# ucb-bar/Accelerated-TinyMPC

Measured on AMD Instinct MI355X. Metric: MPC solves/sec (batched quadrotor nx=12,nu=4,N=30), higher is better.
Workload: dtype f32; 1 GPU; quadrotor_tracking batched 65536 instances per GPU, cold-start tiny_solve, early_exit (tol 1e-3, max_iter 100); nx=12, nu=4, N=30, instances_per_gpu=65536, instances_total=65536, parallelism=batch-shard x1, world_size_seen=1, backend=none (single process), kernel=tile16<12,4,30,exact>, max_iters=85

## Files before the change

accelerated-tinympc_amd/csrc/admm_tile16.hip:

```cpp
#include "rowlane_math.h"
#include <cstdlib>

namespace tinympc
{

typedef float f32x16 __attribute__((ext_vector_type(16)));
#ifndef TINY_T16_ABLATE
#define TINY_T16_ABLATE 0
#endif
#ifndef TINY_T16_CQ
#define TINY_T16_CQ 1
#endif
#ifndef TINY_T16_BADDR
#define TINY_T16_BADDR 1
#endif
#ifndef TINY_T16_PADTAB
#define TINY_T16_PADTAB 1
#endif
#ifndef TINY_T16_XPOSE
#define TINY_T16_XPOSE 1
#endif
#ifndef TINY_T16_SCHED
#define TINY_T16_SCHED 1
#endif
#ifndef TINY_T16_LINES
#define TINY_T16_LINES 1
#endif
#ifndef TINY_T16_STAMP
#define TINY_T16_STAMP 0
#endif

#if TINY_T16_ABLATE == 1
__device__ __forceinline__ f32x4 t16_fake4(float a, float b, f32x4 c) { c[0] += a; c[1] += b; c[2] += a; c[3] += b; return c; }
#define TINY_MFMA4(a, b, c) t16_fake4((a), (b), (c))
#define TINY_MFMA1(a, b, c) __builtin_amdgcn_mfma_f32_16x16x1f32((a), (b), (c), 0, 0, 0)
#else
#define TINY_MFMA4(a, b, c) __builtin_amdgcn_mfma_f32_16x16x4f32((a), (b), (c), 0, 0, 0)
#define TINY_MFMA1(a, b, c) __builtin_amdgcn_mfma_f32_16x16x1f32((a), (b), (c), 0, 0, 0)
#endif

template <int V>
__device__ __forceinline__ void gather12(float (&t)[12], const f32x16 &p0, const f32x16 &p1, const f32x16 &p2)
{
#pragma unroll
    for (int b = 0; b < 4; b++)
    {
        t[b] = p0[4 * b + V];
        t[4 + b] = p1[4 * b + V];
        t[8 + b] = p2[4 * b + V];
    }
}
template <int V>
__device__ __forceinline__ void gather4(float (&t)[4], const f32x16 &p)
{
#pragma unroll
    for (int b = 0; b < 4; b++) t[b] = p[4 * b + V];
}

typedef float f32x2 __attribute__((ext_vector_type(2)));
template <int B>
__device__ __forceinline__ f32x4 blk(const f32x16 &p) { return __builtin_shufflevector(p, p, 4 * B, 4 * B + 1, 4 * B + 2, 4 * B + 3); }
__device__ __forceinline__ void gather12v(f32x4 (&t)[12], const f32x16 &p0, const f32x16 &p1, const f32x16 &p2)
{
    t[0] = blk<0>(p0); t[1] = blk<1>(p0); t[2] = blk<2>(p0); t[3] = blk<3>(p0);
    t[4] = blk<0>(p1); t[5] = blk<1>(p1); t[6] = blk<2>(p1); t[7] = blk<3>(p1);
    t[8] = blk<0>(p2); t[9] = blk<1>(p2); t[10] = blk<2>(p2); t[11] = blk<3>(p2);
}
__device__ __forceinline__ void gather4v(f32x4 (&t)[4], const f32x16 &p)
{
    t[0] = blk<0>(p); t[1] = blk<1>(p); t[2] = blk<2>(p); t[3] = blk<3>(p);
}
template <int LO, int CNT, int NN>
__device__ __forceinline__ f32x4 tree_sum4(const f32x4 (&t)[NN])
{
    if constexpr (CNT == 1) return t[LO];
    else
    {
        constexpr int H = CNT / 2;
        return tree_sum4<LO, H>(t) + tree_sum4<LO + H, CNT - H>(t);
    }
}
template <int PLO, int PCNT, int L, int NN>
__device__ __forceinline__ f32x4 ptree_sum4(const f32x4 (&t)[NN])
{
    if constexpr (PCNT == 1) return t[4 * PLO + L];
    else
    {
        constexpr int H = PCNT / 2;
        return ptree_sum4<PLO, H, L>(t) + ptree_sum4<PLO + H, PCNT - H, L>(t);
    }
}
template <int PLAN, int NN>
__device__ __forceinline__ f32x4 reduce4(const f32x4 (&t)[NN])
{
    if constexpr (NN == 1) return t[0];
    else if constexpr (PLAN == PLAN_SEQ)
    {
        f32x4 acc = t[0];
#pragma unroll
        for (int k = 1; k < NN; k++) acc = acc + t[k];
        return acc;
    }
    else if constexpr (PLAN == PLAN_TREE) return tree_sum4<0, NN>(t);
    else
    {
        static_assert(NN % 4 == 0, "packed VEC plan: whole packets only");
        constexpr int NPK = NN / 4;
        const f32x4 s0 = ptree_sum4<0, NPK, 0>(t), s1 = ptree_sum4<0, NPK, 1>(t), s2 = ptree_sum4<0, NPK, 2>(t), s3 = ptree_sum4<0, NPK, 3>(t);
        return (s0 + s2) + (s1 + s3);
    }
}

template <bool EXACT>
struct TileMath
{
    static constexpr int NX = 12, NU = 4;
    using PL = RowPlans<NX, NU>;
    float A1[3], A2, A3[3], A45, AP[3];
    f32x16 negz;

    __device__ __forceinline__ void load(const float *mats, int g, int c)
    {
        const float *m = mats + 4 * (c & 3) + (c >> 2);
#pragma unroll
        for (int ch = 0; ch < 3; ch++)
        {
            A1[ch] = m[(4 * ch + g) * 16];
            A3[ch] = m[(NX + NU + 4 * ch + g) * 16];
            AP[ch] = m[(2 * NX + 2 * NU + 1 + 4 * ch + g) * 16];
        }
        A2 = m[(NX + g) * 16];
        A45 = m[(2 * NX + NU + g) * 16];
#pragma unroll
        for (int e = 0; e < 16; e++) negz[e] = -0.f;
    }

    struct InFlight
    {
        f32x16 p0, p1, p2, pk;
        f32x4 acc;
    };

    __device__ __forceinline__ void lqr_issue(const float (&s)[3], InFlight &F) const
    {
        if constexpr (EXACT)
        {
            F.p0 = TINY_MFMA1(A1[0], s[0], negz); F.p1 = TINY_MFMA1(A1[1], s[1], negz); F.p2 = TINY_MFMA1(A1[2], s[2], negz);
        }
        else
        {
            f32x4 acc = {-0.f, -0.f, -0.f, -0.f};
            acc = TINY_MFMA4(A1[0], s[0], acc);
            acc = TINY_MFMA4(A1[1], s[1], acc);
            F.acc = TINY_MFMA4(A1[2], s[2], acc);
        }
    }
    __device__ __forceinline__ void lqr_finish(const InFlight &F, float di, float &un, float (&xn)[3]) const
    {
        if constexpr (EXACT)
        {
            static_assert(PL::FWD_XA == PL::FWD_U, "x rows and the u row of a lane are summed in one order (both SEQ for nx = 12, nu = 4)");
            f32x4 t[12];
            gather12v(t, F.p0, F.p1, F.p2);
            const f32x4 acc = reduce4<PL::FWD_XA>(t);
            un = -acc[3] - di;
            const f32x16 pb = TINY_MFMA1(A2, un, negz);
            f32x4 t2[4];
            gather4v(t2, pb);
            const f32x4 xn4 = acc + reduce4<PL::FWD_XB>(t2);
            xn[0] = xn4[0]; xn[1] = xn4[1]; xn[2] = xn4[2];
        }
        else
        {
            un = F.acc[3] - di;
            const f32x4 acc = TINY_MFMA4(A2, un, F.acc);
            xn[0] = acc[0]; xn[1] = acc[1]; xn[2] = acc[2];
        }
    }
    __device__ __forceinline__ void lqr(const float (&s)[3], float di, float &un, float (&xn)[3]) const
    {
        InFlight F;
        lqr_issue(s, F);
        lqr_finish(F, di, un, xn);
    }

    __device__ __forceinline__ void riccati_issue(const float (&p)[3], const f32x4 &lin, InFlight &F) const
    {
        if constexpr (EXACT)
        {
            F.p0 = TINY_MFMA1(A3[0], p[0], negz); F.p1 = TINY_MFMA1(A3[1], p[1], negz); F.p2 = TINY_MFMA1(A3[2], p[2], negz);
            F.pk = TINY_MFMA1(A45, lin[3], negz);
        }
        else
        {
            f32x4 acc = lin;
            acc = TINY_MFMA4(A3[0], p[0], acc);
            acc = TINY_MFMA4(A3[1], p[1], acc);
            F.acc = TINY_MFMA4(A3[2], p[2], acc);
        }
    }
    __device__ __forceinline__ void riccati_finish(const InFlight &F, const f32x4 &lin, float (&pn)[3], float &dd) const
    {
        if constexpr (EXACT)
        {
            f32x4 t4[12];
            gather12v(t4, F.p0, F.p1, F.p2);
            const f32x4 wv = lin + reduce4<PL::BWD_PA>(t4);
            float t[12];
            gather12<3>(t, F.p0, F.p1, F.p2);
            const float wv3 = lin[3] + reduce<PL::BWD_TMP>(t);
            const f32x16 pq = TINY_MFMA1(A45, wv3, negz);
            f32x4 tk4[4];
            gather4v(tk4, F.pk);
            const f32x4 pn4 = wv - reduce4<PL::BWD_PK>(tk4);
            pn[0] = pn4[0]; pn[1] = pn4[1]; pn[2] = pn4[2];
            float tk[4];
            gather4<3>(tk, pq); dd = reduce<PL::BWD_D>(tk);
        }
        else
        {
            const f32x4 nz = {-0.f, -0.f, -0.f, -0.f};
            const f32x4 dq = TINY_MFMA4(A45, F.acc[3], nz);
            const f32x4 acc = TINY_MFMA4(A45, lin[3], F.acc);
            pn[0] = acc[0]; pn[1] = acc[1]; pn[2] = acc[2];
            dd = dq[3];
        }
    }
    __device__ __forceinline__ void riccati(const float (&p)[3], const f32x4 &lin, float (&pn)[3], float &dd) const
    {
        InFlight F;
        riccati_issue(p, lin, F);
        riccati_finish(F, lin, pn, dd);
    }

    __device__ __forceinline__ void terminal(const float (&xr)[3], float (&pt)[3]) const
    {
        if constexpr (EXACT)
        {
            const f32x16 p0 = TINY_MFMA1(AP[0], xr[0], negz), p1 = TINY_MFMA1(AP[1], xr[1], negz), p2 = TINY_MFMA1(AP[2], xr[2], negz);
            float t[12];
            gather12<0>(t, p0, p1, p2); pt[0] = -reduce<PL::TERM>(t);
            gather12<1>(t, p0, p1, p2); pt[1] = -reduce<PL::TERM>(t);
            gather12<2>(t, p0, p1, p2); pt[2] = -reduce<PL::TERM>(t);
        }
        else
        {
            f32x4 acc = {-0.f, -0.f, -0.f, -0.f};
            acc = TINY_MFMA4(AP[0], xr[0], acc);
            acc = TINY_MFMA4(AP[1], xr[1], acc);
            acc = TINY_MFMA4(AP[2], xr[2], acc);
            pt[0] = -acc[0]; pt[1] = -acc[1]; pt[2] = -acc[2];
        }
    }
};

__device__ __forceinline__ float tile_inst_max(float v)
{
    v = fmaxf(v, __shfl_xor(v, 16));
    v = fmaxf(v, __shfl_xor(v, 32));
    return v;
}

__device__ __forceinline__ void acc_put(float &dst, float val) { asm volatile("v_accvgpr_write_b32 %0, %1" : "+a"(dst) : "v"(val)); }
__device__ __forceinline__ float acc_get(const float &src)
{
    float r;
    asm volatile("v_accvgpr_read_b32 %0, %1" : "=v"(r) : "a"(src));
    return r;
}
__device__ __forceinline__ void acc_init(float &dst, float val) { asm volatile("v_accvgpr_write_b32 %0, %1" : "=a"(dst) : "v"(val)); }

typedef __attribute__((address_space(3))) float4 lds_float4;
__device__ __forceinline__ void masked_forward_update(unsigned long long m, float (&a)[4], const f32x4 &tp, float (&bo)[4], const f32x4 &old,
                                                      unsigned sn_addr, const f32x4 &t)
{
    unsigned long long sx;
    asm volatile("s_and_saveexec_b64 %[sx], %[m]\n\t"
                 "v_sub_f32 %[a0], %[p0], %[t0]\n\tv_sub_f32 %[a1], %[p1], %[t1]\n\tv_sub_f32 %[a2], %[p2], %[t2]\n\tv_sub_f32 %[a3], %[p3], %[t3]\n\t"
                 "v_accvgpr_write_b32 %[b0], %[o0]\n\tv_accvgpr_write_b32 %[b1], %[o1]\n\tv_accvgpr_write_b32 %[b2], %[o2]\n\tv_accvgpr_write_b32 %[b3], %[o3]\n\t"
                 "ds_write_b128 %[ad], %[tv]\n\t"
                 "s_mov_b64 exec, %[sx]"
                 : [sx] "=&s"(sx), [a0] "+v"(a[0]), [a1] "+v"(a[1]), [a2] "+v"(a[2]), [a3] "+v"(a[3]), [b0] "+a"(bo[0]), [b1] "+a"(bo[1]),
                   [b2] "+a"(bo[2]), [b3] "+a"(bo[3])
                 : [m] "s"(m), [p0] "v"(tp[0]), [p1] "v"(tp[1]), [p2] "v"(tp[2]), [p3] "v"(tp[3]), [t0] "v"(t[0]), [t1] "v"(t[1]), [t2] "v"(t[2]),
                   [t3] "v"(t[3]), [o0] "v"(old[0]), [o1] "v"(old[1]), [o2] "v"(old[2]), [o3] "v"(old[3]), [ad] "v"(sn_addr), [tv] "v"(t)
                 : "memory", "scc");
}
__device__ __forceinline__ void masked_backward_update(unsigned long long m, float (&pl)[3], float &dr, const float (&pn)[3], float dd)
{
    unsigned long long sx;
    asm volatile("s_and_saveexec_b64 %[sx], %[m]\n\t"
                 "v_accvgpr_write_b32 %[p0], %[n0]\n\tv_accvgpr_write_b32 %[p1], %[n1]\n\tv_accvgpr_write_b32 %[p2], %[n2]\n\tv_mov_b32 %[d], %[dd]\n\t"
                 "s_mov_b64 exec, %[sx]"
                 : [sx] "=&s"(sx), [p0] "+a"(pl[0]), [p1] "+a"(pl[1]), [p2] "+a"(pl[2]), [d] "+v"(dr)
                 : [m] "s"(m), [n0] "v"(pn[0]), [n1] "v"(pn[1]), [n2] "v"(pn[2]), [dd] "v"(dd)
                 : "scc");
}

__device__ __forceinline__ void masked_restore_slack(unsigned long long m, const float (&bo)[4], unsigned sn_addr)
{
    const f32x4 tv = {acc_get(bo[0]), acc_get(bo[1]), acc_get(bo[2]), acc_get(bo[3])};
    unsigned long long sx;
    asm volatile("s_and_saveexec_b64 %[sx], %[m]\n\t"
                 "ds_write_b128 %[ad], %[tv]\n\t"
                 "s_mov_b64 exec, %[sx]"
                 : [sx] "=&s"(sx)
                 : [m] "s"(m), [ad] "v"(sn_addr), [tv] "v"(tv)
                 : "memory", "scc");
}

template <bool EXACT>
__device__ __forceinline__ f32x4 lin_cost4(const f32x4 &cq, const f32x4 &rho4, const f32x4 &t1)
{
    if constexpr (EXACT) return cq - rho4 * t1;
    else return __builtin_elementwise_fma(-rho4, t1, cq);
}

__device__ __forceinline__ f32x4 t16_transpose4(const f32x4 &r)
{
    typedef unsigned u32x2 __attribute__((ext_vector_type(2)));
    const u32x2 a = __builtin_amdgcn_permlane32_swap(__float_as_uint(r[0]), __float_as_uint(r[2]), false, false);
    const u32x2 b = __builtin_amdgcn_permlane32_swap(__float_as_uint(r[1]), __float_as_uint(r[3]), false, false);
    const u32x2 lo = __builtin_amdgcn_permlane16_swap(a[0], b[0], false, false);
    const u32x2 hi = __builtin_amdgcn_permlane16_swap(a[1], b[1], false, false);
    return f32x4{__uint_as_float(lo[0]), __uint_as_float(lo[1]), __uint_as_float(hi[0]), __uint_as_float(hi[1])};
}

constexpr int TILE16_WAVES = 4;
constexpr int TILE16_MAX_TABLE_ROWS = 512;

__device__ __forceinline__ void t16_pair_lines(const f32x4 &e, const f32x4 &o, f32x4 &lo8, f32x4 &hi8)
{
#pragma unroll
    for (int k = 0; k < 4; k++)
    {
        lo8[k] = __int_as_float(__builtin_amdgcn_update_dpp(__float_as_int(e[k]), __float_as_int(o[k]), 0x128, 0xf, 0xc, false));
        hi8[k] = __int_as_float(__builtin_amdgcn_update_dpp(__float_as_int(o[k]), __float_as_int(e[k]), 0x128, 0xf, 0x3, false));
    }
}

#if TINY_T16_STAMP && !defined(TINY_T16_PI_UNIT)
constexpr int T16_STAMP_TILES = 32;
__device__ unsigned long long *t16_stamp_buf;
__device__ int t16_stamp_slots;
__device__ __forceinline__ void t16_stamp(int wslot, int k, int field, unsigned long long v)
{
    unsigned long long *const buf = t16_stamp_buf;
    if (buf && wslot < t16_stamp_slots && k < T16_STAMP_TILES && (threadIdx.x & 63) == 0) buf[((size_t)wslot * T16_STAMP_TILES + k) * 4 + field] = v;
}
#define T16_STAMP(k, field, v) t16_stamp((int)blockIdx.x * TILE16_WAVES + (int)(threadIdx.x >> 6), (k), (field), (v))
#else
#define T16_STAMP(k, field, v) ((void)0)
#endif

__device__ __forceinline__ void t16_dma_row(unsigned on, const float *sbase, unsigned voff, unsigned lds_dst, float after)
{
    asm volatile("s_cmp_eq_u32 %0, 0\n\ts_cbranch_scc1 1f\n\ts_mov_b32 m0, %3\n\ts_nop 0\n\tglobal_load_lds_dwordx4 %1, %2\n1:"
                 : : "s"(on), "v"(voff), "s"(sbase), "s"(lds_dst), "v"(after) : "memory", "scc");
}
__device__ __forceinline__ void t16_dma_row2(unsigned on, const float *sbase, unsigned voff, unsigned lds_dst, float after0, float after1)
{
    asm volatile("s_cmp_eq_u32 %0, 0\n\ts_cbranch_scc1 1f\n\ts_mov_b32 m0, %3\n\ts_nop 0\n\tglobal_load_lds_dwordx4 %1, %2\n\t"
                 "s_add_u32 m0, m0, 0x3f0\n\ts_nop 0\n\tglobal_load_lds_dwordx4 %1, %2 offset:16\n1:"
                 : : "s"(on), "v"(voff), "s"(sbase), "s"(lds_dst), "v"(after0), "v"(after1) : "memory", "scc");
}
__device__ __forceinline__ void t16_dma_img2(unsigned on, const float *sbase, unsigned voff, unsigned lds_dst, float after0, float after1)
{
    asm volatile("s_cmp_eq_u32 %0, 0\n\ts_cbranch_scc1 1f\n\ts_mov_b32 m0, %3\n\ts_nop 0\n\tglobal_load_lds_dwordx4 %1, %2\n\t"
                 "global_load_lds_dwordx4 %1, %2 offset:1024\n1:"
                 : : "s"(on), "v"(voff), "s"(sbase), "s"(lds_dst), "v"(after0), "v"(after1) : "memory", "scc");
}
__device__ __forceinline__ void t16_wait_vm(int k)
{
    if (k == 0) asm volatile("s_waitcnt vmcnt(0)" ::: "memory");
    else if (k == 1) asm volatile("s_waitcnt vmcnt(1)" ::: "memory");
    else if (k == 2) asm volatile("s_waitcnt vmcnt(2)" ::: "memory");
    else if (k == 3) asm volatile("s_waitcnt vmcnt(3)" ::: "memory");
    else if (k == 4) asm volatile("s_waitcnt vmcnt(4)" ::: "memory");
    else if (k == 5) asm volatile("s_waitcnt vmcnt(5)" ::: "memory");
    else if (k == 6) asm volatile("s_waitcnt vmcnt(6)" ::: "memory");
    else if (k == 7) asm volatile("s_waitcnt vmcnt(7)" ::: "memory");
    else asm volatile("s_waitcnt vmcnt(8)" ::: "memory");
}
constexpr int t16_ring_b(bool XR) { return XR ? 3 : 4; }
constexpr int t16_ring_x(bool BR) { return BR ? 4 : 6; }
constexpr int T16_RING_B = 2048, T16_RING_X = 1024;

template <int N, bool EXACT, bool COLD, bool MPC = false, bool BR = false, bool XR = false>
__global__ __launch_bounds__(WAVE * TILE16_WAVES, 1) void admm_tile16_kernel(const RowParams P)
{
    static_assert(!(MPC && (BR || XR)), "the closed loop on chip is instantiated for batch-shared bounds and a shared / windowed reference");
    constexpr int NX = 12, NU = 4;
    const int lane = threadIdx.x & 63, wv = threadIdx.x >> 6, g = lane >> 4, c = lane & 15;
    const int ntiles = (P.batch + 15) >> 4;
    const float rho = P.rho;
    const f32x4 rho4 = {rho, rho, rho, rho};

    extern __shared__ __attribute__((aligned(16))) float4 lds4_base[];
    float4 *const lds4 = lds4_base;
    float4 *const sn0 = lds4 + wv * (N * WAVE) + lane;
    constexpr int DB = t16_ring_b(XR), DX = t16_ring_x(BR);
    const unsigned ringsB = (P.pi_flags & 1u) ? DB : 2, ringsX = (P.pi_flags & 2u) ? DX : 1;
    const unsigned bnd_f4 = BR ? TILE16_WAVES * ringsB * (T16_RING_B / 16) : 2 * N * 4;
    float4 *const blo = lds4 + TILE16_WAVES * N * WAVE, *const bhi = blo + N * 4, *const tab0 = blo + bnd_f4;
    float4 *const tab = tab0;
    const int tab_rows = P.xref_mode == 1 ? P.table_rows : N;
    const float *tab_src = P.xref_mode == 1 ? P.xref_table : P.xref;
    unsigned dmaB = 0, dmaX = 0;
    if constexpr (BR)
    {
        const unsigned ring = (unsigned)(size_t)(lds_float4 *)blo + wv * (ringsB * T16_RING_B);
        dmaB = __builtin_amdgcn_readfirstlane(ring);
    }
    else
    {
        for (int e = threadIdx.x; e < N * 16; e += WAVE * TILE16_WAVES)
        {
            const float2 lh = reinterpret_cast<const float2 *>(P.bounds)[e];
            const int i = e >> 4, r = e & 15;
            reinterpret_cast<float *>(&blo[i * 4 + (r & 3)])[r >> 2] = lh.x;
            reinterpret_cast<float *>(&bhi[i * 4 + (r & 3)])[r >> 2] = lh.y;
        }
    }
    if constexpr (XR)
    {
        const unsigned ring = (unsigned)(size_t)(lds_float4 *)tab0 + wv * (ringsX * T16_RING_X);
        dmaX = __builtin_amdgcn_readfirstlane(ring);
    }
    else
    {
        for (int e = threadIdx.x; e < (tab_rows + N - 1) * 16; e += WAVE * TILE16_WAVES)
        {
            const int er = (e >> 4) < tab_rows ? (e >> 4) : tab_rows - 1;
            float val = tab_src[er * 16 + (e & 15)];
            if (TINY_T16_CQ) val = -(val * ((e & 15) < NX ? P.mats[(2 * NX + 2 * NU) * 16 + (e & 15)] : 1.f));
            reinterpret_cast<float *>(&tab[(e >> 4) * 4 + (e & 3)])[(e & 15) >> 2] = val;
        }
    }
    if constexpr (!BR || !XR) __syncthreads();

    TileMath<EXACT> M;
    M.load(P.mats, g, c);
    f32x4 qv;
#pragma unroll
    for (int v = 0; v < 3; v++) qv[v] = P.mats[(2 * NX + 2 * NU) * 16 + 4 * v + g];
    qv[3] = 1.f;
    constexpr bool CQ = TINY_T16_CQ && !XR;
    auto cost_of = [&](const f32x4 &xr) { return CQ ? xr : -(xr * qv); };

    constexpr bool DQ = COLD && !MPC;
    int qinc = 1;
    if constexpr (DQ)
    {
        const unsigned tail_stride = (P.pi_flags >> 8) & 0xffu;
        if (tail_stride && (((unsigned)blockIdx.x * TILE16_WAVES + (unsigned)wv) % tail_stride) == 0u) qinc = 0x10000;
        qinc = __builtin_amdgcn_readfirstlane(qinc);
    }
#if TINY_T16_STAMP
    int stamp_k = 0;
#else
    constexpr int stamp_k = 0;
#endif
    for (;;)
    {
    int slot = 0;
    if (lane == 0) slot = atomicAdd(P.n_unsolved + 1, qinc);
    slot = __builtin_amdgcn_readfirstlane(slot);
    T16_STAMP(stamp_k, 0, __builtin_amdgcn_s_memrealtime());
    T16_STAMP(stamp_k, 3, ~0ull);
    if (DQ && ntiles <= 32768)
    {
        const int qh = slot & 0xffff, qt = (int)((unsigned)slot >> 16);
        if (qh + qt >= ntiles) break;
        slot = qinc == 1 ? qh : ntiles - 1 - qt;
    }
    else if (slot >= ntiles) break;
    int ozt;
    asm volatile("s_mov_b32 %0, 0" : "=s"(ozt));
    float4 *const sn = sn0 + ozt;
    float4 *const lds4 = lds4_base + ozt;
    int tile = slot;
    if (P.order) tile = P.order[slot];
    const bool tile_ok = tile >= 0 && tile < ntiles;
    T16_STAMP(stamp_k, 3, (unsigned long long)(unsigned)tile);
    constexpr bool GM = COLD && !MPC && !BR && !XR;
    int inst = tile * 16 + c;
    if constexpr (GM)
        if (P.inst_map) inst = P.inst_map[(tile_ok ? tile : 0) * 16 + c];
    auto in_batch = [&](int i) { return GM ? (unsigned)i < (unsigned)P.batch : i < P.batch; };
    const bool valid = tile_ok && in_batch(inst);
    const int inst_a = valid ? inst : P.batch - 1;

    float a[N][4];
    float dr[N], bo[N][4], pl[N][3];
    auto dual4 = [&](int i) { return f32x4{a[i][0], a[i][1], a[i][2], a[i][3]}; };
    const int ebase = (inst_a * N) * 16 + g;
    int wstart = 0;
    if (P.xref_mode == 1) wstart = P.xref_start[inst_a];
    const bool zdual = COLD || (P.duals_zero != 0);

    if constexpr (COLD)
    {
        const float4 z4 = make_float4(0.f, 0.f, 0.f, 0.f);
#pragma unroll
        for (int i = 0; i < N; i++)
        {
            a[i][0] = a[i][1] = a[i][2] = a[i][3] = 0.f;
#pragma unroll
            for (int v = 0; v < 4; v++) acc_init(bo[i][v], 0.f);
            sn[i * WAVE] = z4;
            acc_init(pl[i][0], 0.f); acc_init(pl[i][1], 0.f); acc_init(pl[i][2], 0.f);
            dr[i] = 0.f;
        }
    }
    else
    {
#pragma unroll
        for (int i = 0; i < N; i++)
        {
            float vzl[4], pdv[4];
#pragma unroll
            for (int v = 0; v < 4; v++)
            {
                const int o = ebase + i * 16 + 4 * v;
                vzl[v] = P.vz[o]; pdv[v] = P.pd[o];
                const float gyv = P.gy[o];
                a[i][v] = zdual ? 0.f : gyv;
                acc_init(bo[i][v], vzl[v]);
            }
            sn[i * WAVE] = make_float4(vzl[0], vzl[1], vzl[2], vzl[3]);
            acc_init(pl[i][0], pdv[0]); acc_init(pl[i][1], pdv[1]); acc_init(pl[i][2], pdv[2]);
            dr[i] = pdv[3];
        }
    }
    float x0[3];
#pragma unroll
    for (int v = 0; v < 3; v++) x0[v] = P.xu[ebase + 4 * v];

    const unsigned onB = BR ? (P.pi_flags & 1u) : 0u, onX = XR ? (P.pi_flags & 2u) : 0u;
    struct PiAddr { unsigned rdB, rdX, voffB, voffX; };
    auto pi_addr = [&](unsigned lane16) {
        const unsigned c16 = lane16 & 0xf0u, gg = lane16 >> 8, cc = c16 >> 4;
        const int ins = tile * 16 + (int)cc;
        const unsigned ia = (unsigned)((tile_ok && ins < P.batch) ? ins : P.batch - 1);
        PiAddr A;
        A.rdB = dmaB + 1024u * (gg >> 1) + c16 + 8u * (gg & 1u);
        A.rdX = dmaX + c16 + 4u * gg;
        A.voffB = ia * P.bounds_inst_stride * 8u + 32u * gg;
        A.voffX = ia * P.xref_inst_stride * 4u + 16u * gg;
        return A;
    };
    const float *const xsrc = P.xref;
    auto load_xref = [&](const float4 *tb, int ws, int i, int gsel = -1) {
        if constexpr (XR)
        {
            unsigned ll = lane;
            asm volatile("" : "+v"(ll));
            const unsigned cc = ll & 15u, gg = ll >> 4;
            if (onX)
            {
                const float *rp = xsrc + ((size_t)((tile_ok ? tile : 0) * N + i) * 64 + cc) * 4 + gg;
                return f32x4{rp[0], rp[64], rp[128], 0.f};
            }
            const int ins = tile * 16 + (int)cc;
            const float *rp = xsrc + (size_t)((tile_ok && ins < P.batch) ? ins : P.batch - 1) * P.xref_inst_stride + i * 16 + gg;
            return f32x4{rp[0], rp[4], rp[8], 0.f};
        }
        else
        {
        int row;
        if constexpr (TINY_T16_PADTAB && !(EXACT && COLD && !MPC && !BR && !XR)) row = (ws < tab_rows - 1 ? ws : tab_rows - 1) + i;
        else { row = ws + i; row = row < tab_rows ? row : tab_rows - 1; }
        const float4 t4 = tb[row * 4 + (gsel >= 0 ? gsel : g)];
        return f32x4{t4.x, t4.y, t4.z, t4.w};
        }
    };
    PiAddr A0 = {0u, 0u, 0u, 0u};
    if constexpr (BR || XR)
    {
        A0 = pi_addr(16u * lane);
        if constexpr (BR) { t16_dma_row2(onB ^ 1u, P.bounds, A0.voffB, dmaB, 0.f, 0.f); t16_dma_row2(onB ^ 1u, P.bounds, A0.voffB + (N - 1) * 128u, dmaB + T16_RING_B, 0.f, 0.f); }
        if constexpr (XR) t16_dma_row((onX >> 1) ^ 1u, xsrc, A0.voffX, dmaX, 0.f);
        asm volatile("s_waitcnt vmcnt(0)" ::: "memory");
    }
    auto load_xref_raw = [&](const float4 *tb, int ws, int i) {
        if constexpr (CQ)
        {
            int row = ws + i;
            row = row < tab_rows ? row : tab_rows - 1;
            const float *rp = tab_src + row * 16 + g;
            return f32x4{rp[0], rp[4], rp[8], 0.f};
        }
        else return load_xref(tb, ws, i);
    };
    float pterm[3];
    {
        const f32x4 xrN4 = load_xref_raw(tab, wstart, N - 1);
        const float xrN[3] = {xrN4[0], xrN4[1], xrN4[2]};
        M.terminal(xrN, pterm);
    }

    int st = TINY_STATUS_UNSOLVED_, itn = 1;
    float r_ps = 0.f, r_pi = 0.f, r_ds = 0.f, r_di = 0.f;
    if (valid && !COLD)
    {
        r_ps = P.res[4 * inst + 0]; r_pi = P.res[4 * inst + 1];
        r_ds = P.res[4 * inst + 2]; r_di = P.res[4 * inst + 3];
    }
    float pN[3] = {0.f, 0.f, 0.f};

    auto backward_sweep = [&](unsigned long long amask, const float4 *snI, const float4 *tabI, int wsI) {
        float p[3] = {pN[0], pN[1], pN[2]};
        auto load_lin = [&](int i, float4 &sl, f32x4 &xr) {
            sl = snI[i * WAVE];
            xr = load_xref(tabI, wsI, i);
        };
        auto make_lin = [&](int i, const float4 &sl, const f32x4 &xr) {
            const f32x4 sni = {sl.x, sl.y, sl.z, sl.w};
            return lin_cost4<EXACT>(cost_of(xr), rho4, sni - dual4(i));
        };
        float4 sl0; f32x4 xr0;
        load_lin(N - 2, sl0, xr0);
        f32x4 lin = make_lin(N - 2, sl0, xr0);
#pragma unroll
        for (int i = N - 2; i >= 0; i--)
        {
            float4 sl_n = make_float4(0.f, 0.f, 0.f, 0.f); f32x4 xr_n = {0.f, 0.f, 0.f, 0.f};
            if (EXACT && i > 0) load_lin(i - 1, sl_n, xr_n);
            typename TileMath<EXACT>::InFlight F;
            M.riccati_issue(p, lin, F);
            if (!EXACT && i > 0) load_lin(i - 1, sl_n, xr_n);
#if TINY_T16_SCHED
            if constexpr (EXACT) __builtin_amdgcn_sched_barrier(0);
#endif
            f32x4 lin_n = lin;
            if (i > 0) lin_n = make_lin(i - 1, sl_n, xr_n);
#if TINY_T16_SCHED
            if constexpr (EXACT) __builtin_amdgcn_sched_barrier(0);
#endif
            float pn[3], dd;
            M.riccati_finish(F, lin, pn, dd);
            masked_backward_update(amask, pl[i], dr[i], pn, dd);
            p[0] = pn[0]; p[1] = pn[1]; p[2] = pn[2];
            lin = lin_n;
        }
    };

    for (int ms = 0;; ++ms)
    {
    if (MPC && ms > 0) { st = TINY_STATUS_UNSOLVED_; itn = 1; }
    bool active = valid && (P.max_iter > 0);
    for (int it = 0; it < P.max_iter; ++it)
    {
        if (!__any(active)) break;
        int oz;
        asm volatile("s_mov_b32 %0, 0" : "=s"(oz));
        float4 *const snI = sn + oz;
        const float4 *bloI = blo + oz, *bhiI = bhi + oz;
        const float4 *const tabI = tab + oz;
        const int wsI = wstart + oz;
        const unsigned long long amask = __ballot(active);
        const unsigned sn_addr = (unsigned)(size_t)(lds_float4 *)snI;
        const unsigned gI = (sn_addr - (unsigned)__builtin_amdgcn_readfirstlane(sn_addr)) >> 8;
        const float4 *const bloG = bloI + gI, *const bhiG = bhiI + gI;
        const float *const bsrcI = P.bounds + oz, *const xsrcI = xsrc + oz;
        unsigned rdBI = 0, rdXI = 0;
        if constexpr (BR || XR)
        {
            const PiAddr AI = pi_addr(sn_addr - __builtin_amdgcn_readfirstlane(sn_addr));
            rdBI = COLD ? AI.rdB : A0.rdB + oz; rdXI = COLD ? AI.rdX : A0.rdX + oz;
        }
        const unsigned sB1 = onB ? T16_RING_B : 0u, sX1 = onX ? T16_RING_X : 0u;
        const unsigned sBlast = onB ? ((N - 1) % DB) * T16_RING_B : T16_RING_B;
        const unsigned lane16I = sn_addr - __builtin_amdgcn_readfirstlane(sn_addr);
        const unsigned timg = (unsigned)(tile_ok ? tile : 0) * (unsigned)N;
        unsigned xw = 0, bw = 0;
        if constexpr (XR) xw = timg * 1024u + (COLD ? lane16I : 16u * lane);
        if constexpr (BR) bw = timg * 2048u + (COLD ? lane16I : 16u * lane);
        auto dma_x = [&](int i, float after) { t16_dma_row(onX, xsrcI, xw + (unsigned)i * 1024u, dmaX + (i % DX) * T16_RING_X, after); };
        auto dma_b = [&](int i, float after0, float after1) { t16_dma_img2(onB, bsrcI, bw + (unsigned)i * 2048u, dmaB + (i % DB) * T16_RING_B, after0, after1); };
        typedef __attribute__((address_space(3))) const f32x2 lds_cfloat2;
        typedef __attribute__((address_space(3))) const float lds_cfloat;
        auto ring_bounds = [&](int i, float4 &lo, float4 &hi) {
            lds_cfloat2 *rp = reinterpret_cast<lds_cfloat2 *>(rdBI + (i == N - 1 ? sBlast : (i % DB) * sB1));
            const f32x2 b0 = rp[0], b1 = rp[32], b2 = rp[64], b3 = rp[96];
            lo = make_float4(b0.x, b1.x, b2.x, b3.x); hi = make_float4(b0.y, b1.y, b2.y, b3.y);
        };
        auto ring_xref = [&](int i) {
            lds_cfloat *rp = reinterpret_cast<lds_cfloat *>(rdXI + (i % DX) * sX1);
            return f32x4{rp[0], rp[64], rp[128], 0.f};
        };
        if constexpr (XR)
        {
#pragma unroll
            for (int k = 0; k < DX; k++) dma_x(N - 2 - k, 0.f);
        }
        if constexpr (BR)
        {
#pragma unroll
            for (int k = 0; k < DB - 1; k++) dma_b(k, 0.f, 0.f);
        }
        float s[3] = {x0[0], x0[1], x0[2]};
        float pri_x = 0.f, dua_x = 0.f, pri_u = 0.f, dua_u = 0.f;
        auto elementwise = [&](int i, const f32x4 &sv, const float4 &lo, const float4 &hi, const float4 &ol) {
            const f32x4 old = {ol.x, ol.y, ol.z, ol.w};
            const f32x4 tp = sv + dual4(i);
            f32x4 t;
            t[0] = __builtin_amdgcn_fmed3f(tp[0], lo.x, hi.x);
            t[1] = __builtin_amdgcn_fmed3f(tp[1], lo.y, hi.y);
            t[2] = __builtin_amdgcn_fmed3f(tp[2], lo.z, hi.z);
            t[3] = __builtin_amdgcn_fmed3f(tp[3], lo.w, hi.w);
            const f32x4 dp = sv - t, dd_ = old - t;
            pri_x = fmaxf(fmaxf(fmaxf(pri_x, fabsf(dp[0])), fabsf(dp[1])), fabsf(dp[2]));
            dua_x = fmaxf(fmaxf(fmaxf(dua_x, fabsf(dd_[0])), fabsf(dd_[1])), fabsf(dd_[2]));
            pri_u = fmaxf(pri_u, fabsf(dp[3]));
            dua_u = fmaxf(dua_u, fabsf(dd_[3]));
            if (i == N - 1)
            {
                const f32x4 an = tp - t;
#pragma unroll
                for (int v = 0; v < 3; v++)
                {
                    const float pn_ = lin_cost<EXACT>(pterm[v], rho, t[v] - an[v]);
                    pN[v] = active ? pn_ : pN[v];
                }
            }
            masked_forward_update(amask, a[i], tp, bo[i], old, sn_addr + i * (WAVE * 16), t);
        };
        f32x4 sv_p = {0.f, 0.f, 0.f, 0.f};
        float4 lo_p = make_float4(0.f, 0.f, 0.f, 0.f), hi_p = lo_p, ol_p = lo_p;
#pragma unroll
        for (int i = 0; i < N; i++)
        {
            float4 lo, hi;
            if constexpr (BR)
            {
                if (i + DB - 1 < N) dma_b(i + DB - 1, lo_p.x, hi_p.w);
                t16_wait_vm(2 * ((N - 1 - i) < (DB - 1) ? (N - 1 - i) : (DB - 1)));
                ring_bounds(i, lo, hi);
            }
            else if constexpr (TINY_T16_BADDR && (COLD || !XR)) { lo = bloG[i * 4]; hi = bhiG[i * 4]; }
            else { lo = bloI[i * 4 + g]; hi = bhiI[i * 4 + g]; }
            const float4 ol = snI[i * WAVE];
            typename TileMath<EXACT>::InFlight F;
            if (i < N - 1) M.lqr_issue(s, F);
#if TINY_T16_SCHED
            if constexpr (EXACT) __builtin_amdgcn_sched_barrier(0);
#endif
            if (i > 0) elementwise(i - 1, sv_p, lo_p, hi_p, ol_p);
            float un = 0.f, xn[3] = {0.f, 0.f, 0.f};
            if (i < N - 1) M.lqr_finish(F, dr[i], un, xn);
            sv_p = f32x4{s[0], s[1], s[2], un};
            lo_p = lo; hi_p = hi; ol_p = ol;
            s[0] = xn[0]; s[1] = xn[1]; s[2] = xn[2];
        }
        elementwise(N - 1, sv_p, lo_p, hi_p, ol_p);
        pri_x = tile_inst_max(pri_x); dua_x = tile_inst_max(dua_x);
        pri_u = tile_inst_max(pri_u); dua_u = tile_inst_max(dua_u);
        bool conv = false;
        if (active)
        {
            itn = it + 1;
            if ((it + 1) % P.check_termination == 0)
            {
                r_ps = pri_x; r_ds = dua_x * rho; r_pi = pri_u; r_di = dua_u * rho;
                conv = (r_ps < P.abs_pri_tol) && (r_pi < P.abs_pri_tol) && (r_ds < P.abs_dua_tol) && (r_di < P.abs_dua_tol);
            }
            if (conv) st = TINY_STATUS_SOLVED_;
        }
        active = active && !conv;
        if (!__any(active)) break;
        if (it == P.max_iter - 1) break;
        {
            float p[3] = {pN[0], pN[1], pN[2]};
            const unsigned long long amask = __ballot(active);
            auto load_lin = [&](int i, float4 &sl, f32x4 &xr) {
                sl = snI[i * WAVE];
                if constexpr (XR) xr = ring_xref(i);
                else xr = load_xref(tabI, wsI, i, TINY_T16_BADDR ? (int)gI : -1);
            };
            auto make_lin = [&](int i, const float4 &sl, const f32x4 &xr) {
                const f32x4 sni = {sl.x, sl.y, sl.z, sl.w};
                return lin_cost4<EXACT>(cost_of(xr), rho4, sni - dual4(i));
            };
            float4 sl0; f32x4 xr0;
            if constexpr (XR) t16_wait_vm(0);
            load_lin(N - 2, sl0, xr0);
            f32x4 lin = make_lin(N - 2, sl0, xr0);
#pragma unroll
            for (int i = N - 2; i >= 0; i--)
            {
                float4 sl_n = make_float4(0.f, 0.f, 0.f, 0.f); f32x4 xr_n = {0.f, 0.f, 0.f, 0.f};
                if constexpr (XR)
                {
                    if (i >= DX) dma_x(i - DX, lin[0]);
                    if (i > 0)
                    {
                        const int hi_j = (i - 2) < (N - 2 - DX) ? (i - 2) : (N - 2 - DX), lo_j = (i - DX) > 0 ? (i - DX) : 0;
                        t16_wait_vm(hi_j >= lo_j ? hi_j - lo_j + 1 : 0);
                    }
                }
                if (EXACT && i > 0) load_lin(i - 1, sl_n, xr_n);
                typename TileMath<EXACT>::InFlight F;
                M.riccati_issue(p, lin, F);
                if (!EXACT && i > 0) load_lin(i - 1, sl_n, xr_n);
#if TINY_T16_SCHED
                if constexpr (EXACT) __builtin_amdgcn_sched_barrier(0);
#endif
                f32x4 lin_n = lin;
                if (i > 0) lin_n = make_lin(i - 1, sl_n, xr_n);
#if TINY_T16_SCHED
                if constexpr (EXACT) __builtin_amdgcn_sched_barrier(0);
#endif
                float pn[3], dd;
                M.riccati_finish(F, lin, pn, dd);
                masked_backward_update(amask, pl[i], dr[i], pn, dd);
                p[0] = pn[0]; p[1] = pn[1]; p[2] = pn[2];
                lin = lin_n;
            }
        }
    }
    if (!MPC || ms + 1 >= P.mpc_steps) break;
    if constexpr (MPC)
    {
        int oz;
        asm volatile("s_mov_b32 %0, 0" : "=s"(oz));
        float4 *const snA = sn + oz;
        const unsigned sn_addr = (unsigned)(size_t)(lds_float4 *)snA;
        const bool solved = st == TINY_STATUS_SOLVED_;
        float un, xn_[3];
        M.lqr(x0, dr[0], un, xn_);
        if (P.u0_traj && valid) P.u0_traj[((long long)ms * P.batch + inst) * NU + g] = un;
        {
            const f32x16 p0 = TINY_MFMA1(M.A1[0], x0[0], M.negz), p1 = TINY_MFMA1(M.A1[1], x0[1], M.negz), p2 = TINY_MFMA1(M.A1[2], x0[2], M.negz);
            const f32x16 pb = TINY_MFMA1(M.A2, un, M.negz);
            f32x4 t[12], t2[4];
            gather12v(t, p0, p1, p2);
            gather4v(t2, pb);
            f32x4 z = {0.f, 0.f, 0.f, 0.f};
            asm volatile("" : "+v"(z));
            f32x4 acc = z + t[0];
#pragma unroll
            for (int k = 1; k < 12; k++) acc = acc + t[k];
            const f32x4 x1 = acc + reduce4<PLAN_SEQ>(t2);
            x0[0] = x1[0]; x0[1] = x1[1]; x0[2] = x1[2];
        }
        const unsigned long long umask = __ballot(valid && !solved);
        if (umask != 0ull) backward_sweep(umask, snA, tab + oz, wstart + oz);
        const unsigned long long smask = __ballot(valid && solved);
#pragma unroll
        for (int i = 0; i < N; i++) masked_restore_slack(smask, bo[i], sn_addr + i * (WAVE * 16));
        if (P.xref_mode == 1)
        {
            wstart += P.window_advance;
            const f32x4 xrN4 = load_xref_raw(tab + oz, wstart, N - 1);
            const float xrN[3] = {xrN4[0], xrN4[1], xrN4[2]};
            M.terminal(xrN, pterm);
        }
#pragma unroll
        for (int i = 0; i < N; i++) a[i][0] = a[i][1] = a[i][2] = a[i][3] = 0.f;
    }
    }
    T16_STAMP(stamp_k, 1, __builtin_amdgcn_s_memrealtime());

    auto inst_of = [&](int col) {
        if constexpr (GM)
        {
            int tl = tile_ok ? tile : 0;
            asm volatile("" : "+s"(tl));
            if (P.inst_map) return P.inst_map[tl * 16 + col];
            return tl * 16 + col;
        }
        else return tile * 16 + col;
    };
    int inst_e = inst, ebase_e = ebase;
    bool valid_e = valid;
    if constexpr (GM)
    {
        unsigned ll = lane;
        asm volatile("" : "+v"(ll));
        inst_e = inst_of((int)(ll & 15u));
        valid_e = tile_ok && in_batch(inst_e);
        ebase_e = ((valid_e ? inst_e : P.batch - 1) * N) * 16 + (int)(ll >> 4);
    }

    if (P.max_iter <= 0)
    {
        if (valid_e && g == 0)
        {
            P.status[inst_e] = TINY_STATUS_UNSOLVED_;
            P.iter[inst_e] = 1;
            atomicAdd(P.n_unsolved, 1);
        }
        T16_STAMP(stamp_k, 2, __builtin_amdgcn_s_memrealtime());
#if TINY_T16_STAMP
        ++stamp_k;
#endif
        continue;
    }

    {
        const bool solved = st == TINY_STATUS_SOLVED_;
        const int c2 = lane >> 2, q2 = lane & 3;
        const int inst2 = inst_of(c2);
        const bool valid2 = tile_ok && in_batch(inst2);
        const int obase2 = ((valid2 ? inst2 : 0) * N) * 16 + 4 * q2;
        typedef float float_ma __attribute__((may_alias));
        typedef f32x4 f32x4_ma __attribute__((may_alias));
        float_ma *const stage_w = reinterpret_cast<float_ma *>(lds4 + wv * (N * WAVE));
        const int rd_off = (c2 * 4 + q2);
        const int obase4 = ebase_e + 3 * g;
        constexpr bool XPOSE = TINY_T16_XPOSE && !(EXACT && !COLD && !MPC);
        auto put = [&](float *dst, int i, const f32x4 &val) {
            if constexpr (XPOSE)
            {
                const f32x4 o = t16_transpose4(val);
                if (valid_e) *reinterpret_cast<f32x4 *>(dst + obase4 + i * 16) = o;
                return;
            }
            float_ma *slot = stage_w + i * (WAVE * 4);
            reinterpret_cast<f32x4_ma *>(slot)[lane] = val;
            asm volatile("" ::: "memory");
            f32x4 o;
            o[0] = slot[rd_off]; o[1] = slot[rd_off + 64]; o[2] = slot[rd_off + 128]; o[3] = slot[rd_off + 192];
            asm volatile("" ::: "memory");
            if (valid2) *reinterpret_cast<f32x4 *>(dst + obase2 + i * 16) = o;
        };
        float s[3] = {x0[0], x0[1], x0[2]};
        if constexpr (XPOSE && TINY_T16_LINES && COLD && !MPC && !BR && !XR)
        {
            auto slack_of = [&](int i) { return reinterpret_cast<const f32x4_ma *>(stage_w + i * (WAVE * 4))[lane]; };
            auto lin_of = [&](int i, const f32x4 &sni) {
                const f32x4 xr = load_xref(tab, wstart, i);
                f32x4 lin = lin_cost4<EXACT>(cost_of(xr), rho4, sni - dual4(i));
                if (i == N - 1) lin[3] = 0.f;
                return lin;
            };
            auto pd_of = [&](int i) { return i == N - 1 ? f32x4{pN[0], pN[1], pN[2], 0.f} : f32x4{acc_get(pl[i][0]), acc_get(pl[i][1]), acc_get(pl[i][2]), dr[i]}; };
            auto vz_of = [&](int i, const f32x4 &sni) {
                f32x4 vzv;
    #pragma unroll
                for (int v = 0; v < 4; v++)
                {
                    const float bov = acc_get(bo[i][v]);
                    vzv[v] = solved ? bov : sni[v];
                }
                return vzv;
            };
            const int instL = inst_of(c & 7), instH = inst_of((c & 7) + 8);
            const bool validL = tile_ok && in_batch(instL), validH = tile_ok && in_batch(instH);
            const int obaseL = (validL ? instL : 0) * (N * 16) + ((c >> 3) << 4) + 4 * g;
            const int offH = ((validH ? instH : 0) - (validL ? instL : 0)) * (N * 16);
            auto put2 = [&](float *dst, int i, const f32x4 &ve, const f32x4 &vo) {
                f32x4 lo8, hi8;
                t16_pair_lines(t16_transpose4(ve), t16_transpose4(vo), lo8, hi8);
                if (validL) *reinterpret_cast<f32x4 *>(dst + obaseL + i * 16) = lo8;
                if (validH) *reinterpret_cast<f32x4 *>(dst + obaseL + offH + i * 16) = hi8;
            };
#pragma unroll
            for (int i = 0; i + 1 < N; i += 2)
            {
                const f32x4 sne = slack_of(i), sno = slack_of(i + 1);
                put2(P.gy, i, dual4(i), dual4(i + 1));
                put2(P.vzn, i, sne, sno);
                put2(P.vz, i, vz_of(i, sne), vz_of(i + 1, sno));
                put2(P.pd, i, pd_of(i), pd_of(i + 1));
                put2(P.qr, i, lin_of(i, sne), lin_of(i + 1, sno));
                float ue = 0.f, xe[3];
                M.lqr(s, dr[i], ue, xe);
                const f32x4 sve = {s[0], s[1], s[2], ue};
                float uo = 0.f, xo[3] = {0.f, 0.f, 0.f};
                if (i + 1 < N - 1) M.lqr(xe, dr[i + 1], uo, xo);
                put2(P.xu, i, sve, f32x4{xe[0], xe[1], xe[2], uo});
                s[0] = xo[0]; s[1] = xo[1]; s[2] = xo[2];
            }
            if constexpr (N % 2 == 1)
            {
                const f32x4 sni = slack_of(N - 1);
                put(P.xu, N - 1, f32x4{s[0], s[1], s[2], 0.f});
                put(P.qr, N - 1, lin_of(N - 1, sni));
                put(P.pd, N - 1, pd_of(N - 1));
                put(P.vz, N - 1, vz_of(N - 1, sni));
                put(P.vzn, N - 1, sni);
                put(P.gy, N - 1, dual4(N - 1));
            }
        }
        else
        {
#pragma unroll
        for (int i = 0; i < N; i++)
        {
            float un = 0.f, xn[3] = {0.f, 0.f, 0.f};
            if (i < N - 1) M.lqr(s, dr[i], un, xn);
            const f32x4 sv = {s[0], s[1], s[2], un};
            const f32x4 sni = reinterpret_cast<const f32x4_ma *>(stage_w + i * (WAVE * 4))[lane];
            const f32x4 xr = load_xref(tab, wstart, i);
            f32x4 lin = lin_cost4<EXACT>(cost_of(xr), rho4, sni - dual4(i));
            if (i == N - 1) lin[3] = 0.f;
            f32x4 pdv = {acc_get(pl[i][0]), acc_get(pl[i][1]), acc_get(pl[i][2]), dr[i]};
            if (i == N - 1) pdv = f32x4{pN[0], pN[1], pN[2], 0.f};
            f32x4 vzv;
#pragma unroll
            for (int v = 0; v < 4; v++)
            {
                const float bov = acc_get(bo[i][v]);
                vzv[v] = solved ? bov : sni[v];
            }
            put(P.xu, i, sv);
            put(P.qr, i, lin);
            put(P.pd, i, pdv);
            put(P.vz, i, vzv);
            put(P.vzn, i, sni);
            put(P.gy, i, dual4(i));
            if constexpr (!XPOSE) reinterpret_cast<f32x4_ma *>(stage_w + i * (WAVE * 4))[lane] = sni;
            s[0] = xn[0]; s[1] = xn[1]; s[2] = xn[2];
        }
        }
        const unsigned long long umask = __ballot(valid_e && !solved);
        if (umask != 0ull)
        {
            const bool unsolved2 = valid2 && ((umask >> c2) & 1ull);
            float p[3] = {pN[0], pN[1], pN[2]};
#pragma unroll
            for (int i = N - 2; i >= 0; i--)
            {
                const f32x4 sni = reinterpret_cast<const f32x4_ma *>(stage_w + i * (WAVE * 4))[lane];
                const f32x4 xr = load_xref(tab, wstart, i);
                const f32x4 lin = lin_cost4<EXACT>(cost_of(xr), rho4, sni - dual4(i));
                float pn[3], dd;
                M.riccati(p, lin, pn, dd);
                if constexpr (XPOSE)
                {
                    const f32x4 o = t16_transpose4(f32x4{pn[0], pn[1], pn[2], dd});
                    if (valid_e && !solved) *reinterpret_cast<f32x4 *>(P.pd + obase4 + i * 16) = o;
                }
                else
                {
                float_ma *slot = stage_w + i * (WAVE * 4);
                reinterpret_cast<f32x4_ma *>(slot)[lane] = f32x4{pn[0], pn[1], pn[2], dd};
                asm volatile("" ::: "memory");
                f32x4 o;
                o[0] = slot[rd_off]; o[1] = slot[rd_off + 64]; o[2] = slot[rd_off + 128]; o[3] = slot[rd_off + 192];
                asm volatile("" ::: "memory");
                if (unsolved2) *reinterpret_cast<f32x4 *>(P.pd + obase2 + i * 16) = o;
                }
                p[0] = pn[0]; p[1] = pn[1]; p[2] = pn[2];
            }
        }
        if (valid_e && g == 0)
        {
            P.res[4 * inst_e + 0] = r_ps; P.res[4 * inst_e + 1] = r_pi;
            P.res[4 * inst_e + 2] = r_ds; P.res[4 * inst_e + 3] = r_di;
            P.status[inst_e] = st;
            P.iter[inst_e] = itn;
            if (!solved) atomicAdd(P.n_unsolved, 1);
        }
        if (MPC && valid)
        {
#pragma unroll
            for (int v = 0; v < 3; v++) P.x0buf[inst * NX + 4 * v + g] = x0[v];
            if (g == 0 && P.xref_mode == 1) P.xref_start[inst] = wstart;
        }
    }
    T16_STAMP(stamp_k, 2, __builtin_amdgcn_s_memrealtime());
#if TINY_T16_STAMP
    ++stamp_k;
#endif
    }
}

#ifdef TINY_T16_ONLY30
#define TINY_FOR_EACH_TILE16(X) X(30)
#else
#define TINY_FOR_EACH_TILE16(X) X(30) X(25) X(20) X(10)
#endif

static inline unsigned t16_tail_stride(const RowParams &P, int ntiles, int nblocks, int asked, bool grouped)
{
    static const int env = [] { const char *e = getenv("TINYMPC_T16_TAIL"); return e ? atoi(e) : -1; }();
    const int forced = asked >= 0 ? asked : env;
    if (ntiles > 32768) return 0u;
    if (forced >= 0) return (P.cold_start && P.mpc_steps <= 1) ? (unsigned)(forced > 255 ? 255 : forced) : 0u;
    if (!P.order || P.mpc_steps > 1 || !P.cold_start) return 0u;
    const int slots = nblocks * TILE16_WAVES;
    if (ntiles < 3 * slots) return 0u;
    if (grouped) return ntiles < 8 * slots ? 12u : 8u;
    return (ntiles >= 4 * slots && ntiles < 8 * slots) ? 4u : 8u;
}

#ifdef TINY_T16_PI_UNIT
size_t tile16_pi_lds_bytes(int N, bool bounds_ring, bool xref_ring, unsigned pi_flags, int table_rows)
{
    const size_t bnd = bounds_ring ? (size_t)TILE16_WAVES * ((pi_flags & 1u) ? t16_ring_b(xref_ring) : 2) * T16_RING_B : (size_t)2 * N * 4 * sizeof(float4);
    const size_t ref = xref_ring ? (size_t)TILE16_WAVES * ((pi_flags & 2u) ? t16_ring_x(bounds_ring) : 1) * T16_RING_X : (size_t)(table_rows + N - 1) * 4 * sizeof(float4);
    return (size_t)TILE16_WAVES * N * WAVE * sizeof(float4) + bnd + ref;
}

hipError_t launch_admm_tile16_pi(int N, bool exact, bool bounds_ring, bool xref_ring, const RowParams &P, hipStream_t stream, int n_cu, int tail)
{
    const int ntiles = (P.batch + 15) / 16;
    if (n_cu <= 0) n_cu = 256;
    const int want = (ntiles + TILE16_WAVES - 1) / TILE16_WAVES, nblocks = want < n_cu ? want : n_cu;
    if (P.mpc_steps > 1 || (!bounds_ring && !xref_ring)) return hipErrorInvalidValue;
    if (P.xref_mode == 1 && P.table_rows < 1) return hipErrorInvalidValue;
    if (!bounds_ring && P.bounds_inst_stride != 0) return hipErrorInvalidValue;
    if (!xref_ring && P.xref_mode != 1 && P.xref_inst_stride != 0) return hipErrorInvalidValue;
    if (xref_ring && P.xref_mode == 1) return hipErrorInvalidValue;
    const size_t lds = tile16_pi_lds_bytes(N, bounds_ring, xref_ring, P.pi_flags, P.xref_mode == 1 ? P.table_rows : N);
    if (lds > 160 * 1024) return hipErrorInvalidValue;
    RowParams Q = P;
    Q.inst_map = nullptr;
    Q.pi_flags = (Q.pi_flags & 0xffu) | (t16_tail_stride(P, ntiles, nblocks, tail, false) << 8);
#define TINY_TILE16_PI_LAUNCH3(NN, EX, BRR, XRR)                                                                           \
    {                                                                                                                      \
        auto kern = P.cold_start ? admm_tile16_kernel<NN, EX, true, false, BRR, XRR> : admm_tile16_kernel<NN, EX, false, false, BRR, XRR>; \
        hipError_t e = hipFuncSetAttribute((const void *)kern, hipFuncAttributeMaxDynamicSharedMemorySize, (int)lds);      \
        if (e != hipSuccess) return e;                                                                                     \
        hipLaunchKernelGGL(kern, dim3(nblocks), dim3(WAVE * TILE16_WAVES), lds, stream, Q);                                \
        return hipGetLastError();                                                                                          \
    }
#define TINY_TILE16_PI_LAUNCH(NN, EX)                                             \
    {                                                                             \
// ... 97 lines not shown
```

Before: 48.00 million solves/s.

## Hoist exec masking to whole forward/backward sweeps in cold exact path

For the exact cold-start non-MPC kernel, the active-lane exec mask is now narrowed once around the whole forward and backward sweeps instead of being saved and restored inside every per-step masked update. The per-step updates become plain asm without exec toggling, and the last add of d_i is fused into the backward-update asm. Explicit s_waitcnt plus sched barriers are inserted ahead of LDS consumers, and the reference-table row clamp is changed for this path. The intent is to remove scalar exec save/restore overhead from the hot loop. The risk is that compiler-generated code inside the narrowed region also runs only on active lanes, and the hand-placed waits may over-serialise.

```diff
diff --git a/accelerated-tinympc_amd/csrc/admm_tile16.hip b/accelerated-tinympc_amd/csrc/admm_tile16.hip
--- a/accelerated-tinympc_amd/csrc/admm_tile16.hip
+++ b/accelerated-tinympc_amd/csrc/admm_tile16.hip
@@ -16,6 +16,12 @@
 #endif
 #ifndef TINY_T16_PADTAB
 #define TINY_T16_PADTAB 1
+#endif
+#ifndef TINY_T16_HEADPAD
+#define TINY_T16_HEADPAD 1
+#endif
+#ifndef TINY_T16_HEADWAIT
+#define TINY_T16_HEADWAIT 1
 #endif
 #ifndef TINY_T16_XPOSE
 #define TINY_T16_XPOSE 1
@@ -199,7 +205,8 @@
             F.acc = TINY_MFMA4(A3[2], p[2], acc);
         }
     }
-    __device__ __forceinline__ void riccati_finish(const InFlight &F, const f32x4 &lin, float (&pn)[3], float &dd) const
+    template <bool SPLIT = false>
+    __device__ __forceinline__ void riccati_finish(const InFlight &F, const f32x4 &lin, float (&pn)[3], float &dd, float *ddb = nullptr) const
     {
         if constexpr (EXACT)
         {
@@ -215,7 +222,13 @@
             const f32x4 pn4 = wv - reduce4<PL::BWD_PK>(tk4);
             pn[0] = pn4[0]; pn[1] = pn4[1]; pn[2] = pn4[2];
             float tk[4];
-            gather4<3>(tk, pq); dd = reduce<PL::BWD_D>(tk);
+            gather4<3>(tk, pq);
+            if constexpr (SPLIT)
+            {
+                static_assert(!SPLIT || PL::BWD_D == PLAN_SEQ, "d_i is summed sequentially: ((t0 + t1) + t2) + t3");
+                dd = (tk[0] + tk[1]) + tk[2]; *ddb = tk[3];
+            }
+            else dd = reduce<PL::BWD_D>(tk);
         }
         else
         {
@@ -297,6 +310,36 @@
                  : "scc");
 }
 
+#pragma clang diagnostic push
+#pragma clang diagnostic ignored "-Winline-asm"
+__device__ __forceinline__ unsigned long long exec_narrow(unsigned long long m)
+{
+    unsigned long long sx;
+    asm volatile("s_and_saveexec_b64 %0, %1" : "=&s"(sx) : "s"(m) : "memory", "scc", "exec");
+    return sx;
+}
+__device__ __forceinline__ void exec_restore(unsigned long long sx) { asm volatile("s_mov_b64 exec, %0" : : "s"(sx) : "memory", "exec"); }
+#pragma clang diagnostic pop
+__device__ __forceinline__ void region_forward_update(float (&a)[4], const f32x4 &tp, float (&bo)[4], const f32x4 &old, unsigned sn_addr, int off,
+                                                      const f32x4 &t)
+{
+    asm volatile("v_sub_f32 %[a0], %[p0], %[t0]\n\tv_sub_f32 %[a1], %[p1], %[t1]\n\tv_sub_f32 %[a2], %[p2], %[t2]\n\tv_sub_f32 %[a3], %[p3], %[t3]\n\t"
+                 "v_accvgpr_write_b32 %[b0], %[o0]\n\tv_accvgpr_write_b32 %[b1], %[o1]\n\tv_accvgpr_write_b32 %[b2], %[o2]\n\tv_accvgpr_write_b32 %[b3], %[o3]\n\t"
+                 "ds_write_b128 %[ad], %[tv] offset:%[off]"
+                 : [a0] "+v"(a[0]), [a1] "+v"(a[1]), [a2] "+v"(a[2]), [a3] "+v"(a[3]), [b0] "+a"(bo[0]), [b1] "+a"(bo[1]), [b2] "+a"(bo[2]),
+                   [b3] "+a"(bo[3])
+                 : [p0] "v"(tp[0]), [p1] "v"(tp[1]), [p2] "v"(tp[2]), [p3] "v"(tp[3]), [t0] "v"(t[0]), [t1] "v"(t[1]), [t2] "v"(t[2]), [t3] "v"(t[3]),
+                   [o0] "v"(old[0]), [o1] "v"(old[1]), [o2] "v"(old[2]), [o3] "v"(old[3]), [ad] "v"(sn_addr), [tv] "v"(t), [off] "i"(off)
+                 : "memory");
+}
+__device__ __forceinline__ void region_backward_update(float (&pl)[3], float &dr, const float (&pn)[3], float dda, float ddb)
+{
+    asm volatile("v_accvgpr_write_b32 %[p0], %[n0]\n\tv_accvgpr_write_b32 %[p1], %[n1]\n\tv_accvgpr_write_b32 %[p2], %[n2]\n\tv_add_f32 %[d], %[da], %[db]"
+                 : [p0] "+a"(pl[0]), [p1] "+a"(pl[1]), [p2] "+a"(pl[2]), [d] "+v"(dr)
+                 : [n0] "v"(pn[0]), [n1] "v"(pn[1]), [n2] "v"(pn[2]), [da] "v"(dda), [db] "v"(ddb));
+}
+__device__ __forceinline__ void region_sub(float &dst, float x, float y) { asm volatile("v_sub_f32 %0, %1, %2" : "+v"(dst) : "v"(x), "v"(y)); }
+
 __device__ __forceinline__ void masked_restore_slack(unsigned long long m, const float (&bo)[4], unsigned sn_addr)
 {
     const f32x4 tv = {acc_get(bo[0]), acc_get(bo[1]), acc_get(bo[2]), acc_get(bo[3])};
@@ -391,6 +434,7 @@
 {
     static_assert(!(MPC && (BR || XR)), "the closed loop on chip is instantiated for batch-shared bounds and a shared / windowed reference");
     constexpr int NX = 12, NU = 4;
+    constexpr bool HEAD = EXACT && COLD && !MPC && !BR && !XR;
     const int lane = threadIdx.x & 63, wv = threadIdx.x >> 6, g = lane >> 4, c = lane & 15;
     const int ntiles = (P.batch + 15) >> 4;
     const float rho = P.rho;
@@ -569,7 +613,7 @@
         else
         {
         int row;
-        if constexpr (TINY_T16_PADTAB && !(EXACT && COLD && !MPC && !BR && !XR)) row = (ws < tab_rows - 1 ? ws : tab_rows - 1) + i;
+        if constexpr (TINY_T16_PADTAB && !(EXACT && COLD && !MPC && !BR && !XR && !TINY_T16_HEADPAD)) row = (ws < tab_rows - 1 ? ws : tab_rows - 1) + i;
         else { row = ws + i; row = row < tab_rows ? row : tab_rows - 1; }
         const float4 t4 = tb[row * 4 + (gsel >= 0 ? gsel : g)];
         return f32x4{t4.x, t4.y, t4.z, t4.w};
@@ -700,9 +744,17 @@
 #pragma unroll
             for (int k = 0; k < DB - 1; k++) dma_b(k, 0.f, 0.f);
         }
+        unsigned long long exec_fw = 0ull;
+        if constexpr (HEAD) exec_fw = exec_narrow(amask);
         float s[3] = {x0[0], x0[1], x0[2]};
         float pri_x = 0.f, dua_x = 0.f, pri_u = 0.f, dua_u = 0.f;
         auto elementwise = [&](int i, const f32x4 &sv, const float4 &lo, const float4 &hi, const float4 &ol) {
+            if constexpr (HEAD && TINY_T16_HEADWAIT)
+            {
+                if (i == N - 1) __builtin_amdgcn_s_waitcnt(0xC07F);
+                else __builtin_amdgcn_s_waitcnt(0xC37F);
+                __builtin_amdgcn_sched_barrier(0);
+            }
             const f32x4 old = {ol.x, ol.y, ol.z, ol.w};
             const f32x4 tp = sv + dual4(i);
             f32x4 t;
@@ -721,10 +773,16 @@
 #pragma unroll
                 for (int v = 0; v < 3; v++)
                 {
+                    if constexpr (HEAD) region_sub(pN[v], pterm[v], rho * (t[v] - an[v]));
+                    else
+                    {
                     const float pn_ = lin_cost<EXACT>(pterm[v], rho, t[v] - an[v]);
                     pN[v] = active ? pn_ : pN[v];
+                    }
                 }
             }
+            if constexpr (HEAD) region_forward_update(a[i], tp, bo[i], old, sn_addr, i * (WAVE * 16), t);
+            else
             masked_forward_update(amask, a[i], tp, bo[i], old, sn_addr + i * (WAVE * 16), t);
         };
         f32x4 sv_p = {0.f, 0.f, 0.f, 0.f};
@@ -755,6 +813,7 @@
             s[0] = xn[0]; s[1] = xn[1]; s[2] = xn[2];
         }
         elementwise(N - 1, sv_p, lo_p, hi_p, ol_p);
+        if constexpr (HEAD) exec_restore(exec_fw);
         pri_x = tile_inst_max(pri_x); dua_x = tile_inst_max(dua_x);
         pri_u = tile_inst_max(pri_u); dua_u = tile_inst_max(dua_u);
         bool conv = false;
@@ -774,6 +833,8 @@
         {
             float p[3] = {pN[0], pN[1], pN[2]};
             const unsigned long long amask = __ballot(active);
+            unsigned long long exec_bw = 0ull;
+            if constexpr (HEAD) exec_bw = exec_narrow(amask);
             auto load_lin = [&](int i, float4 &sl, f32x4 &xr) {
                 sl = snI[i * WAVE];
                 if constexpr (XR) xr = ring_xref(i);
@@ -808,16 +869,28 @@
                 if constexpr (EXACT) __builtin_amdgcn_sched_barrier(0);
 #endif
                 f32x4 lin_n = lin;
+                if constexpr (HEAD && TINY_T16_HEADWAIT)
+                    if (i > 0) { __builtin_amdgcn_s_waitcnt(0xC07F); __builtin_amdgcn_sched_barrier(0); }
                 if (i > 0) lin_n = make_lin(i - 1, sl_n, xr_n);
 #if TINY_T16_SCHED
                 if constexpr (EXACT) __builtin_amdgcn_sched_barrier(0);
 #endif
                 float pn[3], dd;
+                if constexpr (HEAD)
+                {
+                    float ddb;
+                    M.template riccati_finish<true>(F, lin, pn, dd, &ddb);
+                    region_backward_update(pl[i], dr[i], pn, dd, ddb);
+                }
+                else
+                {
                 M.riccati_finish(F, lin, pn, dd);
                 masked_backward_update(amask, pl[i], dr[i], pn, dd);
+                }
                 p[0] = pn[0]; p[1] = pn[1]; p[2] = pn[2];
                 lin = lin_n;
             }
+            if constexpr (HEAD) exec_restore(exec_bw);
         }
     }
     if (!MPC || ms + 1 >= P.mpc_steps) break;
```

After: 50.29 million solves/s, median of 6. 1.05x the previous value.
